# emmanuel-marty/zultra

Hardware: NVIDIA B200
Metric: input MB/s (zultra compression hot path, byte-identical to CPU zultra) (higher is better)
Workload: dtype u8

## Files before the change

### zultra_b200/csrc/zb_pipeline.h

```cpp
#ifndef ZB_PIPELINE_H
#define ZB_PIPELINE_H
#include "zb_rt.h"
#include <vector>
#include <algorithm>
#ifndef ZB_EMU
#include <cuda_pipeline.h>
#endif

#ifndef ZB_CG
#define ZB_CG 1024
#endif
#ifndef ZB_CP
#define ZB_CP 1024
#endif
#define ZB_CD 2048
#define ZB_WU 384
#define ZB_TOKI 256
#define ZB_NH 320
#define ZB_MAXSB 64
#define ZB_MAXNODES 64
#define ZB_MF_TILE_MAX 16384

struct ZbWinDesc {
   uint32_t in_off;
// ... 129 lines not shown
struct ZbPipe {
   zb_stream_t st;
   ZbHostBuf hin, hout;
#ifndef ZB_EMU
   ZbStager stager;
   int device = 0;
#endif
   int nwin = 0, nstream = 0;
   uint32_t P = 0;
   std::vector<ZbWinDesc> h_win;
   std::vector<uint32_t> h_wbase;
   ZbBuf<ZbWinDesc> win; ZbBuf<uint32_t> wbase;
   ZbBuf<uint8_t> in;
   const uint8_t *in_ptr = 0;
   ZbBuf<uint64_t> keyA, keyB; ZbBuf<uint32_t> valA, valB, rank, sa, actA, actB, tmpA, tmpB, scratch;
   ZbBuf<uint32_t> sa_lcp;
   ZbBuf<uint32_t> counters;
   ZbBuf<ZbTileDesc> tiles, units, groups; ZbBuf<uint32_t> tile_iv, tile_pd, tile_cnt, tile_q, unit_words, unit_cnt, group_words, group_cnt, filt_seg;
   ZbBuf<zb_match_t> match; ZbBuf<uint16_t> glen, goff;
   ZbBuf<uint16_t> exitoff, exitc; ZbBuf<uint32_t> gentry, gtokcnt, gtokbase, tokpos, wtok;
   ZbBuf<uint32_t> wtokbase, wintbase; ZbBuf<int> ph;
   std::vector<uint32_t> h_gchunk_first; ZbBuf<uint32_t> gchunk_first, gchunk_win;
   ZbBuf<ZbNode> nodesA, nodesB; ZbBuf<int> nodehist; ZbBuf<uint16_t> chk_stat; ZbBuf<uint8_t> chk_flag; ZbBuf<int> chk_delta; ZbBuf<uint32_t> chk_node;
   ZbBuf<uint32_t> wsplit; ZbBuf<uint32_t> wnsplit, wsubcnt, wsubbase;
   ZbBuf<ZbSub> sub; ZbBuf<ZbSubTabs> tabs; ZbBuf<uint32_t> dchunk_sub, pchunk_sub;
   ZbBuf<zb_match_t> best; ZbBuf<int16_t> sig_true, sig_warm, sig_new; ZbBuf<uint8_t> dok; ZbBuf<uint32_t> dbad;
   ZbBuf<uint32_t> pentry, pbits, cand ; ZbBuf<uint16_t> dpfar;
   int cp = ZB_CP;
   ZbBuf<int> dreach;
   ZbBuf<uint32_t> out; ZbBuf<ZbStreamOut> sout;
   std::vector<ZbStreamOut> h_sout;
   int nsub = 0;
   bool sa_exact = false;
   int parse_cd = 0, parse_wu = ZB_WU;
   int mf_ts_min = ZB_TS_MIN, mf_ts_mul = ZB_TS_MUL;
   int stat_sa_rounds = 0, stat_redo = 0, stat_ub = 0, stat_tiles = 0;
   double t_stage[8];

   void release_all();
   void setup(const std::vector<ZbWinDesc> &wins, const uint8_t *h_in, size_t in_bytes, bool in_is_device);
   void stage_sa();
   void stage_match(uint32_t tile_main);
   void stage_greedy();
   void stage_split();
   void stage_parse();
   void stage_emit(const std::vector<ZbStreamOut> &streams) { stage_emit_prepare(); stage_emit_finish(streams); }
   void stage_emit_prepare();
   void stage_emit_finish(const std::vector<ZbStreamOut> &streams, uint32_t *ext_words = 0);
   void phase_maps(const std::vector<ZbStreamOut> &streams, unsigned long long *bits_out);
   std::vector<ZbStreamOut> plan;
   ZbBuf<uint32_t> ck_tab, ck_part; ZbBuf<uint64_t> ck_rng; bool ck_tab_ready = false;
   void stage_checksum(int kind, const std::vector<uint64_t> &range_off, const std::vector<uint64_t> &range_len, std::vector<uint32_t> &sums, uint32_t init_first);
};

ZB_HD int zb_find_win(const uint32_t *wbase, int nwin, uint32_t g) {
   int lo = 0, hi = nwin - 1;
   while (lo < hi) { int mid = (lo + hi + 1) >> 1; if (wbase[mid] <= g) lo = mid; else hi = mid - 1; }
   return lo;
}

inline void ZbPipe::setup(const std::vector<ZbWinDesc> &wins, const uint8_t *h_in, size_t in_bytes, bool in_is_device) {
   h_win = wins; nwin = (int)wins.size();
   h_wbase.assign(nwin + 1, 0);
   for (int w = 0; w < nwin; w++) h_wbase[w + 1] = h_wbase[w] + wins[w].len;
   P = h_wbase[nwin];
   win.need(nwin); wbase.need(nwin + 1); counters.need(64);
   if (!in_is_device) in.need(in_bytes + 16);
   if (zb_failed()) return;
   zb_h2d(st, win.p, h_win.data(), sizeof(ZbWinDesc) * nwin);
   zb_h2d(st, wbase.p, h_wbase.data(), 4 * (nwin + 1));
   if (in_is_device) in_ptr = h_in;
   else {
      if (h_in) {
#ifndef ZB_EMU
         if (in_bytes >= ((size_t)8 << 20) && ZbStager::pageable(h_in)) { zb_sync(st); if (!stager.copy(0, in.p, (void *)h_in, in_bytes, device)) zb_cuda_fail(cudaErrorUnknown); }
         else
#endif
         zb_h2d(st, in.p, h_in, in_bytes);
      }
      in_ptr = in.p;
   }
}

#define ZB_SA_LOCAL 32

ZB_HD void zb_sa_key(const uint8_t *t, uint32_t i, uint32_t len, uint32_t d, uint64_t &w, uint32_t &tl) {
   const uint32_t rem = len - i;
   tl = rem < d + 9 ? rem : d + 9;
#ifdef __CUDA_ARCH__
   if ((uint64_t)i + d + 12 <= len) {
      const uintptr_t a = (uintptr_t)(t + i + d);
      const uint32_t *pa = (const uint32_t *)(a & ~(uintptr_t)3);
      const uint32_t sh = (uint32_t)(a & 3) << 3;
      const uint32_t x0 = __funnelshift_r(pa[0], pa[1], sh), x1 = __funnelshift_r(pa[1], pa[2], sh);
      w = ((uint64_t)__byte_perm(x0, 0, 0x0123) << 32) | __byte_perm(x1, 0, 0x0123);
      return;
   }
#endif
   uint64_t x = 0;
   for (uint32_t b = 0; b < 8; b++) x = (x << 8) | ((uint64_t)i + d + b < len ? t[i + d + b] : 0u);
   w = x;
}

inline void ZbPipe::stage_sa() {
   const long n = P;
   keyA.need(n); keyB.need(n); valA.need(n); valB.need(n); rank.need(n); sa.need(n); actA.need(n); actB.need(n); tmpA.need(n + 1); tmpB.need(n + 1);
   sa_lcp.need(n);
   scratch.need(zb_sort_scratch_words(n) + zb_scan_scratch_words(n) + 64);
   if (zb_failed()) return;
   int wb = 0; while ((1L << wb) < nwin) wb++;
   int nbytes = (64 - wb) / 8; if (nbytes > 7) nbytes = 7;
   {
      static const int nb_env = getenv("ZULTRA_CUDA_SA_NBYTES") ? atoi(getenv("ZULTRA_CUDA_SA_NBYTES")) : 0;
      if (nb_env >= 3 && nb_env < nbytes) nbytes = nb_env;
   }
   const uint8_t *T = in_ptr; const ZbWinDesc *wd = win.p; const uint32_t *wbs = wbase.p; const int nw = nwin;
   uint64_t *kA = keyA.p; uint32_t *vA = valA.p;
   zb_tag("sa_keys");
   zb_launch(st, n, ZB_LAMBDA(long g) {
      int w = zb_find_win(wbs, nw, (uint32_t)g);
      uint32_t i = (uint32_t)g - wbs[w], len = wd[w].len;
      const uint8_t *t = T + wd[w].in_off;
      uint64_t k = 0;
      for (int b = 0; b < nbytes; b++) k = (k << 8) | (i + b < len ? t[i + b] : 0);
      kA[g] = ((uint64_t)w << (8 * nbytes)) | k;
      vA[g] = (uint32_t)g;
   }, 256);
   zb_sort_pairs(st, keyA.p, valA.p, keyB.p, valB.p, n, 0, 8 * nbytes + wb, scratch.p);
   uint32_t *head = tmpA.p, *grp = tmpB.p, *rk = rank.p, *SA = sa.p, *act = actA.p, *act2 = actB.p, *cnt = counters.p;
   const int kbits = 8 * nbytes;
   zb_tag("sa_group");
   zb_launch(st, n, ZB_LAMBDA(long jl) {
      const uint32_t j = (uint32_t)jl;
      const uint64_t key = kA[j];
      uint32_t gh = j, step = 1;
      while (gh >= step && kA[gh - step] == key) { gh -= step; step <<= 1; }
      long lo = gh >= step ? (long)(gh - step) : -1L;
      while ((long)gh - lo > 1) { const uint32_t mid = (uint32_t)((lo + (long)gh) >> 1); if (kA[mid] == key) gh = mid; else lo = mid; }
      const uint32_t g = vA[j];
      if ((long)gh + ZB_SA_LOCAL < n && kA[gh + ZB_SA_LOCAL] == key) { SA[j] = g; rk[g] = gh; head[j] = 1u; return; }
      uint32_t ge = j + 1;
      while ((long)ge < n && kA[ge] == key) ge++;
      if (ge - gh == 1) { SA[j] = g; rk[g] = j; head[j] = 0u; return; }
      const int w = (int)(key >> kbits);
      const uint32_t base = wbs[w], len = wd[w].len;
      const uint8_t *t = T + wd[w].in_off;
      uint64_t kw; uint32_t kt;
      zb_sa_key(t, g - base, len, (uint32_t)nbytes, kw, kt);
      uint32_t less = 0, eq_before = 0, eq = 0;
      for (uint32_t y = gh; y < ge; y++) {
         if (y == j) continue;
         uint64_t yw; uint32_t yt;
         zb_sa_key(t, vA[y] - base, len, (uint32_t)nbytes, yw, yt);
         if (yw < kw || (yw == kw && yt < kt)) less++;
         else if (yw == kw && yt == kt) { eq++; if (y < j) eq_before++; }
      }
      const uint32_t p = gh + less + eq_before;
      SA[p] = g; rk[g] = gh + less; head[p] = eq ? 1u : 0u;
   }, 256);
   zb_exclusive_sum(st, head, grp, n, cnt, scratch.p);
   zb_launch(st, n, ZB_LAMBDA(long j) { if (head[j]) act[grp[j]] = (uint32_t)j; }, 256);
   uint32_t m = 0;
   zb_d2h(st, &m, cnt, 4); zb_sync(st);
   int rank_bits = 1; while ((1L << rank_bits) < n) rank_bits++;
   uint64_t *kB = keyB.p; uint32_t *vB = valB.p;
   stat_sa_rounds = 0;
   uint32_t maxwin = 0;
   for (int w = 0; w < nwin; w++) maxwin = std::max(maxwin, h_win[w].len);
   int r2_bits = 1; while ((1L << r2_bits) < (long)maxwin + 512) r2_bits++;
   const bool packed_keys = !sa_exact;
   for (uint32_t h = (uint32_t)nbytes; m > 0 && (sa_exact || h < ZB_MAX_MATCH); h <<= 1) {
      stat_sa_rounds++;
      const long mm = m;
      zb_tag("sa_round_keys");
      if (packed_keys) {
         zb_launch(st, mm, ZB_LAMBDA(long a) {
            uint32_t j = act[a], g = SA[j];
            int w = zb_find_win(wbs, nw, g);
            uint32_t wend = wbs[w + 1];
            uint32_t r2;
            if ((uint64_t)g + h < wend) r2 = (rk[g + h] - wbs[w]) + 512u;
            else r2 = wend - g;
            kA[a] = ((uint64_t)rk[g] << r2_bits) | r2;
            vA[a] = g;
         }, 256);
         zb_sort_pairs(st, keyA.p, valA.p, keyB.p, valB.p, mm, 0, r2_bits + rank_bits, scratch.p);
      } else {
      zb_launch(st, mm, ZB_LAMBDA(long a) {
         uint32_t j = act[a], g = SA[j];
         int w = zb_find_win(wbs, nw, g);
         uint32_t wend = wbs[w + 1];
         uint32_t r2;
         if ((uint64_t)g + h < wend) r2 = (rk[g + h] - wbs[w]) + (1u << 22);
         else r2 = wend - g;
         kA[a] = ((uint64_t)rk[g] << 32) | r2;
         vA[a] = g;
      }, 256);
      zb_sort_pairs(st, keyA.p, valA.p, keyB.p, valB.p, mm, 0, 23, scratch.p);
      zb_sort_pairs(st, keyA.p, valA.p, keyB.p, valB.p, mm, 32, 32 + rank_bits, scratch.p);
      }
      zb_launch(st, mm, ZB_LAMBDA(long a) { head[a] = (a == 0 || kA[a] != kA[a - 1]) ? (uint32_t)a : 0u; SA[act[a]] = vA[a]; }, 256);
      zb_inclusive_max(st, head, grp, mm, scratch.p);
      zb_launch(st, mm, ZB_LAMBDA(long a) {
         const uint32_t ga = grp[a];
         rk[vA[a]] = act[ga];
         bool is_head = ga == (uint32_t)a;
         bool next_head = (a + 1 == mm) || grp[a + 1] == (uint32_t)(a + 1);
         head[a] = (is_head && next_head) ? 0u : 1u;
      }, 256);
      zb_exclusive_sum(st, head, (uint32_t *)kB, mm, cnt, scratch.p);
      {
         const uint32_t *dst = (const uint32_t *)kB;
         zb_launch(st, mm, ZB_LAMBDA(long a) { if (head[a]) act2[dst[a]] = act[a]; }, 256);
      }
      zb_d2h(st, &m, cnt, 4); zb_sync(st);
      std::swap(act, act2);
      (void)vB;
      if (h > (1u << 23)) break;
   }
   uint32_t *out = sa_lcp.p;
   zb_tag("lcp_pack");
   zb_launch(st, n, ZB_LAMBDA(long j) {
      uint32_t g = SA[j];
      int w = zb_find_win(wbs, nw, (uint32_t)j);
      uint32_t base = wbs[w], len = wd[w].len;
      uint32_t i = g - base;
      uint32_t l = 0;
      if ((uint32_t)j != base) {
         uint32_t q = SA[j - 1] - base;
         const uint8_t *t = T + wd[w].in_off;
         uint32_t lim = len - (i > q ? i : q);
         if (lim > ZB_MAX_MATCH) lim = ZB_MAX_MATCH;
#ifdef __CUDA_ARCH__
         if (wd[w].in_off + (i < q ? i : q) >= 4) {
            while (l + 8 <= lim) {
               const uintptr_t a = (uintptr_t)(t + i + l), b = (uintptr_t)(t + q + l);
               const uint32_t *pa = (const uint32_t *)(a & ~(uintptr_t)3), *pb = (const uint32_t *)(b & ~(uintptr_t)3);
               const uint32_t x = __funnelshift_r(pa[0], pa[1], (uint32_t)(a & 3) << 3) ^ __funnelshift_r(pb[0], pb[1], (uint32_t)(b & 3) << 3);
               if (x) { l += (uint32_t)(__ffs((int)x) - 1) >> 3; lim = l; break; }
               l += 4;
            }
         }
// ... 2655 lines not shown
```

### zultra_b200/csrc/zb_prims.cu

```cuda
#include "zb_rt.h"

void zb_cuda_fail(cudaError_t e) {
   (void)e;
   g_zb_cuda_error = 1;
}
thread_local int g_zb_cuda_error = 0;
long long g_zb_launches = 0;

#include <vector>
#include <string>
#include <map>
#include <mutex>
int g_zb_prof_on = 0;
struct ZbProfRec { std::string tag; cudaEvent_t a, b; };
static std::vector<ZbProfRec> g_prof;
static std::mutex g_prof_mu;
static thread_local const char *g_next_tag = 0;
static thread_local ZbProfRec g_cur;
void zb_tag(const char *tag) { g_next_tag = tag; }
void zb_prof_begin(int line, cudaStream_t st) {
   if (g_next_tag) g_cur.tag = g_next_tag; else { char b[32]; snprintf(b, sizeof b, "L%d", line); g_cur.tag = b; }
   g_next_tag = 0;
   cudaEventCreate(&g_cur.a); cudaEventCreate(&g_cur.b);
   cudaEventRecord(g_cur.a, st);
// ... 195 lines not shown
      __syncwarp();
   }
   __syncthreads();
   uint32_t tot = 0;
#pragma unroll
   for (int w = 0; w < RS_WARPS; w++) { uint32_t t = cnt[w][tid]; cnt[w][tid] = tot; tot += t; }
   uint32_t inc = tot;
#pragma unroll
   for (int d = 1; d < 32; d <<= 1) { uint32_t o = __shfl_up_sync(0xffffffffu, inc, d); if (lane >= d) inc += o; }
   if (lane == 31) wsum[warp] = inc;
   __syncthreads();
   uint32_t woff = 0;
#pragma unroll
   for (int w = 0; w < RS_WARPS; w++) if (w < warp) woff += wsum[w];
   const uint32_t ds = woff + inc - tot;
   dstart[tid] = ds;
   gbase[tid] = gb - ds;
   __syncthreads();
#pragma unroll
   for (int k = 0; k < RS_ITEMS; k++) {
      const long idx = base + k * 32 + lane;
      if (idx < n) {
         const uint32_t d = (uint32_t)(key[k] >> shift) & mask;
         const uint32_t lp = dstart[d] + cnt[warp][d] + rk[k];
         skey[lp] = key[k]; sval[lp] = val[k];
      }
   }
   __syncthreads();
   const long tile_n = n - (long)blockIdx.x * RS_TILE < RS_TILE ? n - (long)blockIdx.x * RS_TILE : RS_TILE;
#pragma unroll
   for (int k = 0; k < RS_ITEMS; k++) {
      const int e = k * RS_THREADS + tid;
      if (e < tile_n) {
         const uint64_t kk = skey[e];
         const uint32_t d = (uint32_t)(kk >> shift) & mask;
         const size_t dst = (size_t)(uint32_t)(gbase[d] + (uint32_t)e);
         kout[dst] = kk;
         vout[dst] = sval[e];
      }
   }
}

size_t zb_sort_scratch_words(long n) {
   long ntiles = (n + RS_TILE - 1) / RS_TILE;
   if (ntiles < 1) ntiles = 1;
   return (size_t)256 * ntiles + zb_scan_scratch_words(256 * ntiles) + 64;
}

void zb_sort_pairs(zb_stream_t st, uint64_t *keys, uint32_t *vals, uint64_t *keys_tmp, uint32_t *vals_tmp, long n, int bit_lo, int bit_hi, uint32_t *scratch) {
   if (n <= 1 || bit_hi <= bit_lo) return;
   const int ntiles = (int)((n + RS_TILE - 1) / RS_TILE);
   uint32_t *hist = scratch;
   uint32_t *scan_scratch = scratch + (size_t)256 * ntiles;
   uint64_t *kin = keys, *kout = keys_tmp;
   uint32_t *vin = vals, *vout = vals_tmp;
   int npass = 0;
   for (int shift = bit_lo; shift < bit_hi; shift += 8, npass++) {
      const int w = (bit_hi - shift) < 8 ? (bit_hi - shift) : 8;
      const uint32_t mask = (1u << w) - 1u;
      PROF_K("rs_hist", st);
      rs_hist_k<<<ntiles, RS_THREADS, 0, st>>>(kin, n, shift, mask, hist, ntiles);
      PROF_E(st);
      scan_impl<OpSum, false>(st, hist, hist, (long)256 * ntiles, 0, scan_scratch);
      PROF_K("rs_scatter", st);
      rs_scatter_k<<<ntiles, RS_THREADS, 0, st>>>(kin, vin, kout, vout, n, shift, mask, hist, ntiles);
      PROF_E(st);
      zb_count_launch(2);
      uint64_t *tk = kin; kin = kout; kout = tk;
      uint32_t *tv = vin; vin = vout; vout = tv;
   }
   ZB_CUDA_CHECK(cudaGetLastError());
   if (npass & 1) {
      ZB_CUDA_CHECK(cudaMemcpyAsync(keys, keys_tmp, (size_t)n * 8, cudaMemcpyDeviceToDevice, st));
      ZB_CUDA_CHECK(cudaMemcpyAsync(vals, vals_tmp, (size_t)n * 4, cudaMemcpyDeviceToDevice, st));
   }
}


#define DS_SEG 4096
#define DS_THREADS 256
#define DS_WORDS (DS_SEG / 32)
#define DS_BROW (DS_WORDS + 1)
#define DS_PROW (DS_WORDS + 2)

__device__ __forceinline__ int ds_find_win(const ZbDistWin *dw, int nwin, uint32_t seg) {
   int lo = 0, hi = nwin - 1;
   while (lo < hi) { const int mid = (lo + hi + 1) >> 1; if (dw[mid].seg_base <= seg) lo = mid; else hi = mid - 1; }
   return lo;
}

template <bool SCATTER>
__global__ void __launch_bounds__(DS_THREADS) unit_dist_k(const uint32_t *sa_lcp, const ZbDistWin *dw, int nwin, int nu_max, uint32_t *segrec, uint32_t *unit_words) {
   extern __shared__ uint32_t ds_sm[];
   uint32_t *bm = ds_sm;
   uint16_t *pre = (uint16_t *)(bm + (size_t)nu_max * DS_BROW);
   uint16_t *lcp = pre + (size_t)nu_max * DS_PROW;
   uint16_t *bmin = lcp + DS_SEG;
   uint32_t *uoff = (uint32_t *)(bmin + DS_WORDS);
   uint32_t *stage = uoff + nu_max + 1;
   const int tid = threadIdx.x, lane = tid & 31, warp = tid >> 5;
   const int w = ds_find_win(dw, nwin, blockIdx.x);
   const ZbDistWin W = dw[w];
   const uint32_t seg = blockIdx.x - W.seg_base, r0 = seg * DS_SEG;
   const uint32_t nr = W.len - r0 < DS_SEG ? W.len - r0 : DS_SEG;
   const int nu = (int)W.nu;
   {
      const size_t tot = (size_t)dw[nwin - 1].sa_base + dw[nwin - 1].len;
      const size_t pf = (size_t)W.sa_base + r0 + (size_t)1024 * DS_SEG + (size_t)tid * 32;
      if (tid < DS_SEG / 32 && pf < tot) asm volatile("prefetch.global.L2 [%0];" :: "l"(sa_lcp + pf));
   }
   if (nu == 1) {
      if (!SCATTER) { if (tid == 0) { segrec[(size_t)blockIdx.x * nu_max * 2] = nr; segrec[(size_t)blockIdx.x * nu_max * 2 + 1] = 0x1ffu | 0x10000u; } }
      else for (uint32_t idx = tid; idx < nr; idx += DS_THREADS) unit_words[(size_t)W.unit_base * (2 * ZB_MAX_OFFSET) + r0 + idx] = __ldg(sa_lcp + W.sa_base + r0 + idx);
      return;
   }
   uint32_t wv[DS_SEG / DS_THREADS];
#pragma unroll
   for (int k = 0; k < DS_SEG / DS_THREADS; k++) {
      const uint32_t idx = (uint32_t)k * DS_THREADS + tid;
      wv[k] = idx < nr ? __ldg(sa_lcp + W.sa_base + r0 + idx) : (0x1ffu << ZB_POS_BITS);
   }
   for (int e = tid; e < nu * DS_BROW; e += DS_THREADS) bm[e] = 0;
   __syncthreads();
#pragma unroll
   for (int k = 0; k < DS_SEG / DS_THREADS; k++) {
      const uint32_t idx = (uint32_t)k * DS_THREADS + tid;
      uint32_t v = wv[k];
      if (idx < nr) {
         const uint32_t p = v & ZB_POS_MASK;
         const int ua = p < W.hist ? 0 : (int)((p - W.hist) >> 15);
         atomicOr(bm + ua * DS_BROW + (idx >> 5), 1u << (idx & 31));
         if (p >= W.hist && ua + 1 < nu) atomicOr(bm + (ua + 1) * DS_BROW + (idx >> 5), 1u << (idx & 31));
      }
      wv[k] = v;
      lcp[idx] = (uint16_t)((v >> ZB_POS_BITS) & 0x1ffu);
   }
   __syncthreads();
   for (int b = warp; b < DS_WORDS; b += DS_THREADS / 32) {
      const uint32_t m = __reduce_min_sync(0xffffffffu, (uint32_t)lcp[b * 32 + lane]);
      if (lane == 0) bmin[b] = (uint16_t)m;
   }
   __syncthreads();
   uint32_t *rec = segrec + (size_t)blockIdx.x * nu_max * 2;
   if (!SCATTER) {
      for (int u = warp; u < nu; u += DS_THREADS / 32) {
         const uint32_t *b = bm + u * DS_BROW;
         uint32_t c = 0; int last = -1;
#pragma unroll
         for (int j = 0; j < DS_WORDS / 32; j++) {
            const uint32_t x = b[j * 32 + lane];
            c += (uint32_t)__popc(x);
            if (x) last = (j * 32 + lane) * 32 + 31 - __clz((int)x);
         }
#pragma unroll
         for (int d = 16; d > 0; d >>= 1) { c += __shfl_xor_sync(0xffffffffu, c, d); last = max(last, __shfl_xor_sync(0xffffffffu, last, d)); }
         uint32_t m = 0x1ffu;
         const int from = last + 1;
         const int fb = (from + 31) >> 5;
         { const int i = from + lane; if (i < fb * 32 && i < DS_SEG) m = lcp[i]; }
         for (int bb = fb + lane; bb < DS_WORDS; bb += 32) m = min(m, (uint32_t)bmin[bb]);
         m = __reduce_min_sync(0xffffffffu, m);
         if (lane == 0) { rec[2 * u] = c; rec[2 * u + 1] = m | (last >= 0 ? 0x10000u : 0u); }
      }
      return;
   }
   for (int u = warp; u < nu; u += DS_THREADS / 32) {
      const uint32_t *b = bm + u * DS_BROW;
      uint32_t run = 0;
#pragma unroll
      for (int j = 0; j < DS_WORDS / 32; j++) {
         const uint32_t c = (uint32_t)__popc(b[j * 32 + lane]);
         uint32_t inc = c;
#pragma unroll
         for (int d = 1; d < 32; d <<= 1) { const uint32_t o = __shfl_up_sync(0xffffffffu, inc, d); if (lane >= d) inc += o; }
         pre[u * DS_PROW + j * 32 + lane] = (uint16_t)(run + inc - c);
         run += __shfl_sync(0xffffffffu, inc, 31);
      }
      if (lane == 0) uoff[u + 1] = run;
   }
   __syncthreads();
   if (tid == 0) { uint32_t acc = 0; uoff[0] = 0; for (int u = 0; u < nu; u++) { const uint32_t c = uoff[u + 1]; uoff[u + 1] = acc + c; acc += c; } }
   __syncthreads();
#pragma unroll
   for (int k = 0; k < DS_SEG / DS_THREADS; k++) {
      const uint32_t idx = (uint32_t)k * DS_THREADS + tid;
      if (idx >= nr) continue;
      const uint32_t p = wv[k] & ZB_POS_MASK;
      const int ua = p < W.hist ? 0 : (int)((p - W.hist) >> 15);
      const int nun = (p >= W.hist && ua + 1 < nu) ? 2 : 1;
      for (int q = 0; q < nun; q++) {
         const int u = ua + q;
         const uint32_t *b = bm + u * DS_BROW;
         const uint32_t wi = idx >> 5, below = b[wi] & ((1u << (idx & 31)) - 1u);
         const uint32_t rank = (uint32_t)pre[u * DS_PROW + wi] + (uint32_t)__popc(below);
         int prev = -1;
         if (below) prev = (int)(wi * 32) + 31 - __clz((int)below);
         else for (int x = (int)wi - 1; x >= 0; x--) { const uint32_t y = b[x]; if (y) { prev = x * 32 + 31 - __clz((int)y); break; } }
         uint32_t m = 0x1ffu;
         const int from = prev + 1, fb = (from + 31) >> 5, lb = (int)(idx >> 5);
         if (fb > lb) { for (int i = from; i <= (int)idx; i++) m = min(m, (uint32_t)lcp[i]); }
         else {
            for (int i = from; i < fb * 32; i++) m = min(m, (uint32_t)lcp[i]);
            for (int bb = fb; bb < lb; bb++) m = min(m, (uint32_t)bmin[bb]);
            for (int i = lb * 32; i <= (int)idx; i++) m = min(m, (uint32_t)lcp[i]);
         }
         if (prev < 0) m = min(m, rec[2 * u + 1]);
         const uint32_t m0 = W.hist + (uint32_t)u * ZB_MAX_OFFSET, ulo = m0 > ZB_MAX_OFFSET ? m0 - ZB_MAX_OFFSET : 0;
         stage[uoff[u] + rank] = (p - ulo) | (m << ZB_POS_BITS);
      }
   }
   __syncthreads();
   for (int u = warp; u < nu; u += DS_THREADS / 32) {
      const uint32_t a = uoff[u], n = uoff[u + 1] - a;
      uint32_t *dst = unit_words + (size_t)(W.unit_base + u) * (2 * ZB_MAX_OFFSET) + rec[2 * u];
      for (uint32_t j = lane; j < n; j += 32) dst[j] = stage[a + j];
   }
}

__global__ void unit_dist_offsets_k(const ZbDistWin *dw, int nwin, int nu_max, uint32_t *segrec, uint32_t *unit_cnt, int total_units) {
   const int g = blockIdx.x * blockDim.x + threadIdx.x;
   if (g >= total_units) return;
   int lo = 0, hi = nwin - 1;
   while (lo < hi) { const int mid = (lo + hi + 1) >> 1; if (dw[mid].unit_base <= (uint32_t)g) lo = mid; else hi = mid - 1; }
   const ZbDistWin W = dw[lo];
   const int u = g - (int)W.unit_base;
   const uint32_t nseg = (W.len + DS_SEG - 1) / DS_SEG;
   uint32_t acc = 0, carry = 0x1ffu;
   for (uint32_t sg = 0; sg < nseg; sg++) {
      uint32_t *rec = segrec + ((size_t)(W.seg_base + sg) * nu_max + u) * 2;
      const uint32_t c = rec[0], th = rec[1];
      rec[0] = acc; rec[1] = carry;
      acc += c;
      const uint32_t tl = th & 0xffffu;
      carry = (th >> 16) ? tl : (tl < carry ? tl : carry);
   }
   unit_cnt[g] = acc;
}

void zb_unit_distribute(zb_stream_t st, const uint32_t *sa_lcp, const ZbDistWin *dw, int nwin, int nseg_total, int total_units, int nu_max, uint32_t *segrec,
                        uint32_t *unit_words, uint32_t *unit_cnt) {
   if (nseg_total <= 0 || total_units <= 0) return;
   const size_t smem = (size_t)nu_max * DS_BROW * 4 + (size_t)nu_max * DS_PROW * 2 + DS_SEG * 2 + DS_WORDS * 2 + ((size_t)nu_max + 1) * 4 + 2 * DS_SEG * 4 + 16;
   ZB_CUDA_CHECK(cudaFuncSetAttribute(unit_dist_k<false>, cudaFuncAttributeMaxDynamicSharedMemorySize, 112 * 1024));
   ZB_CUDA_CHECK(cudaFuncSetAttribute(unit_dist_k<true>, cudaFuncAttributeMaxDynamicSharedMemorySize, 112 * 1024));
   PROF_K("mf_unit_dist", st);
   unit_dist_k<false><<<nseg_total, DS_THREADS, smem - 2 * DS_SEG * 4, st>>>(sa_lcp, dw, nwin, nu_max, segrec, unit_words);
   unit_dist_offsets_k<<<(total_units + 127) / 128, 128, 0, st>>>(dw, nwin, nu_max, segrec, unit_cnt, total_units);
   unit_dist_k<true><<<nseg_total, DS_THREADS, smem, st>>>(sa_lcp, dw, nwin, nu_max, segrec, unit_words);
   PROF_E(st);
   zb_count_launch(3);
   ZB_CUDA_CHECK(cudaGetLastError());
}
```

Measured before the change: 1507.

## Resolve small suffix-array groups in shared memory with multi-step local refinement

```diff
diff --git a/zultra_b200/csrc/zb_pipeline.h b/zultra_b200/csrc/zb_pipeline.h
--- a/zultra_b200/csrc/zb_pipeline.h
+++ b/zultra_b200/csrc/zb_pipeline.h
@@ -235,7 +235,9 @@
    }
 }
 
-#define ZB_SA_LOCAL 32
+#define ZB_SA_LOCAL 64
+#define ZB_SA_SPAN 1024
+#define ZB_SA_STEPS 2
 
 ZB_HD void zb_sa_key(const uint8_t *t, uint32_t i, uint32_t len, uint32_t d, uint64_t &w, uint32_t &tl) {
    const uint32_t rem = len - i;
@@ -254,6 +256,197 @@
    for (uint32_t b = 0; b < 8; b++) x = (x << 8) | ((uint64_t)i + d + b < len ? t[i + d + b] : 0u);
    w = x;
 }
+
+#ifndef ZB_EMU
+struct ZbSaRec { uint64_t w; uint32_t st; uint32_t g; };
+#define ZB_SA_LT 256
+#define ZB_SA_CAP (ZB_SA_SPAN + ZB_SA_LOCAL - 1)
+#define ZB_SA_SPT (ZB_SA_SPAN / ZB_SA_LT)
+#define ZB_SA_IPT ((ZB_SA_CAP + ZB_SA_LT - 1) / ZB_SA_LT)
+
+__device__ __forceinline__ bool zb_sa_rec_less(const ZbSaRec &a, const ZbSaRec &b) {
+   if ((a.st >> 9) != (b.st >> 9)) return a.st < b.st;
+   if (a.w != b.w) return a.w < b.w;
+   return a.st < b.st;
+}
+
+template <bool MAX> __device__ __forceinline__ uint32_t zb_sa_cta_scan(uint32_t v, uint32_t *ws, uint32_t &tot) {
+   const int lane = threadIdx.x & 31, warp = threadIdx.x >> 5;
+   uint32_t inc = v;
+#pragma unroll
+   for (int o = 1; o < 32; o <<= 1) { const uint32_t y = __shfl_up_sync(0xffffffffu, inc, o); if (lane >= o) inc = MAX ? max(inc, y) : inc + y; }
+   uint32_t ex = __shfl_up_sync(0xffffffffu, inc, 1);
+   if (lane == 0) ex = 0;
+   if (lane == 31) ws[warp] = inc;
+   __syncthreads();
+   uint32_t pre = 0, all = 0;
+#pragma unroll
+   for (int w = 0; w < ZB_SA_LT / 32; w++) {
+      const uint32_t x = ws[w];
+      if (w < warp) pre = MAX ? max(pre, x) : pre + x;
+      all = MAX ? max(all, x) : all + x;
+   }
+   __syncthreads();
+   tot = all;
+   return MAX ? max(pre, ex) : pre + ex;
+}
+
+__global__ void __launch_bounds__(ZB_SA_LT) zb_sa_local_k(const uint64_t *kA, const uint32_t *vA, long n, const uint8_t *T, const ZbWinDesc *wd,
+                                                         const uint32_t *wbs, int nw, uint32_t nb, uint32_t *SA, uint32_t *rk, uint32_t *head) {
+   extern __shared__ __align__(16) ZbSaRec zb_sar[];
+   ZbSaRec *A = zb_sar, *B = zb_sar + ZB_SA_CAP;
+   uint16_t *pos = (uint16_t *)(zb_sar + 2 * ZB_SA_CAP);
+   uint16_t *grp = pos + ZB_SA_CAP;
+   __shared__ uint32_t ws[ZB_SA_LT / 32], s_end, s_tail;
+   const int tid = threadIdx.x;
+   const uint32_t s0 = blockIdx.x * ZB_SA_SPAN, s1 = (uint32_t)min((long)s0 + ZB_SA_SPAN, n);
+   __shared__ uint16_t gsz[ZB_SA_SPAN];
+   __shared__ uint8_t gstart[ZB_SA_SPAN];
+   __shared__ uint32_t s_gh0, s_large0;
+   const uint32_t sl = s1 - s0, p0 = tid * ZB_SA_SPT;
+   for (int p = tid; p < ZB_SA_CAP; p += ZB_SA_LT) grp[p] = 0xffffu;
+   if (tid == 0) {
+      s_end = sl; s_tail = 0xffffu; s_gh0 = s0; s_large0 = 0;
+      const uint64_t key = kA[s0];
+      if (s0 > 0 && kA[s0 - 1] == key) {
+         uint32_t gh = s0, step = 1;
+         while (gh >= step && kA[gh - step] == key) { gh -= step; step <<= 1; }
+         long lo = gh >= step ? (long)(gh - step) : -1L;
+         while ((long)gh - lo > 1) { const uint32_t mid = (uint32_t)((lo + (long)gh) >> 1); if (kA[mid] == key) gh = mid; else lo = mid; }
+         s_gh0 = gh; s_large0 = (long)gh + ZB_SA_LOCAL < n && kA[gh + ZB_SA_LOCAL] == key;
+      }
+   }
+   uint64_t key[ZB_SA_SPT];
+   uint32_t startm = 0, last_start = 0;
+#pragma unroll
+   for (int i = 0; i < ZB_SA_SPT; i++) {
+      const uint32_t p = p0 + i, j = s0 + p;
+      key[i] = p < sl ? kA[j] : 0;
+      const bool st = p < sl && (j == 0 || (i ? key[i - 1] : kA[j - 1]) != key[i]);
+      gstart[p] = st;
+      if (st) { startm |= 1u << i; last_start = p + 1; }
+   }
+   uint32_t unused;
+   uint32_t cur = zb_sa_cta_scan<true>(last_start, ws, unused);
+#pragma unroll
+   for (int i = 0; i < ZB_SA_SPT; i++) {
+      if (!((startm >> i) & 1u)) continue;
+      const uint32_t p = p0 + i, lim = min(p + ZB_SA_LOCAL + 1, sl);
+      uint32_t q = p + 1;
+      while (q < lim && !gstart[q]) q++;
+      uint32_t sz = q - p;
+      if (q == p + ZB_SA_LOCAL + 1) sz = ZB_SA_LOCAL + 1;
+      else if (q == sl && (long)s1 < n && kA[s1] == key[i]) {
+         const uint32_t gh = s0 + p;
+         if ((long)gh + ZB_SA_LOCAL < n && kA[gh + ZB_SA_LOCAL] == key[i]) sz = ZB_SA_LOCAL + 1;
+         else {
+            uint32_t e = s1, st2 = 1;
+            while ((long)e + st2 < n && kA[e + st2] == key[i]) { e += st2; st2 <<= 1; }
+            long hi = min((long)e + st2, n);
+            while (hi - (long)e > 1) { const uint32_t mid = (uint32_t)(((long)e + hi) >> 1); if (kA[mid] == key[i]) e = mid; else hi = mid; }
+            sz = (uint32_t)hi - gh; s_end = (uint32_t)hi - s0; s_tail = p;
+         }
+      }
+      gsz[p] = (uint16_t)sz;
+   }
+   __syncthreads();
+#pragma unroll
+   for (int i = 0; i < ZB_SA_SPT; i++) {
+      const uint32_t p = p0 + i, j = s0 + p;
+      if (p >= sl) break;
+      if ((startm >> i) & 1u) cur = p + 1;
+      const uint32_t g = vA[j];
+      if (cur == 0) {
+         if (s_large0) { SA[j] = g; rk[g] = s_gh0; head[j] = 1u; }
+         continue;
+      }
+      const uint32_t sz = gsz[cur - 1], gh = s0 + cur - 1;
+      if (sz > ZB_SA_LOCAL) { SA[j] = g; rk[g] = gh; head[j] = 1u; }
+      else if (sz == 1) { SA[j] = g; rk[g] = j; head[j] = 0u; }
+      else grp[p] = (uint16_t)(cur - 1);
+   }
+   __syncthreads();
+   const uint32_t np = s_end;
+   for (uint32_t p = sl + tid; p < np; p += ZB_SA_LT) grp[p] = (uint16_t)s_tail;
+   __syncthreads();
+   uint32_t na;
+   {
+      uint32_t c = 0;
+#pragma unroll
+      for (int i = 0; i < ZB_SA_IPT; i++) { const uint32_t p = tid * ZB_SA_IPT + i; if (p < np && grp[p] != 0xffffu) c++; }
+      uint32_t o = zb_sa_cta_scan<false>(c, ws, na);
+#pragma unroll
+      for (int i = 0; i < ZB_SA_IPT; i++) {
+         const uint32_t p = tid * ZB_SA_IPT + i;
+         if (p < np && grp[p] != 0xffffu) { A[o].w = 0; A[o].st = (uint32_t)grp[p] << 9; A[o].g = vA[s0 + p]; pos[o] = (uint16_t)p; o++; }
+      }
+      __syncthreads();
+   }
+   for (uint32_t d = nb, step = 0; na > 0; d += 8, step++) {
+      for (uint32_t k = tid; k < na; k += ZB_SA_LT) {
+         ZbSaRec &r = A[k];
+         const int w = zb_find_win(wbs, nw, r.g);
+         uint64_t kw; uint32_t tl;
+         zb_sa_key(T + wd[w].in_off, r.g - wbs[w], wd[w].len, d, kw, tl);
+         r.w = kw; r.st = (r.st & ~511u) | tl;
+      }
+      __syncthreads();
+      for (uint32_t k = tid; k < na; k += ZB_SA_LT) {
+         const ZbSaRec r = A[k];
+         const uint32_t run = r.st >> 9;
+         uint32_t lo = k;
+         while (lo > 0 && (A[lo - 1].st >> 9) == run) lo--;
+         uint32_t before = 0;
+         for (uint32_t y = lo; y < na && (A[y].st >> 9) == run; y++) {
+            const ZbSaRec x = A[y];
+            before += zb_sa_rec_less(x, r) || (y < k && x.w == r.w && x.st == r.st);
+         }
+         B[lo + before] = r;
+      }
+      __syncthreads();
+      { ZbSaRec *t = A; A = B; B = t; }
+      const bool last = step + 1 == ZB_SA_STEPS;
+      const uint32_t full = d + 9;
+      uint32_t run_last = 0, ntied = 0, tpm = 0, tnm = 0;
+#pragma unroll
+      for (int i = 0; i < ZB_SA_IPT; i++) {
+         const uint32_t k = tid * ZB_SA_IPT + i;
+         if (k < na) {
+            const ZbSaRec r = A[k];
+            const bool tied = (r.st & 511u) == full;
+            const bool tp = tied && k > 0 && A[k - 1].st == r.st && A[k - 1].w == r.w;
+            const bool tn = tied && k + 1 < na && A[k + 1].st == r.st && A[k + 1].w == r.w;
+            if (!tp) run_last = k;
+            if (tp || tn) ntied++;
+            tpm |= (uint32_t)tp << i; tnm |= (uint32_t)tn << i;
+         }
+      }
+      uint32_t unused, nt;
+      uint32_t rs = zb_sa_cta_scan<true>(run_last, ws, unused);
+      uint32_t o = zb_sa_cta_scan<false>(last ? 0u : ntied, ws, nt);
+      uint32_t kg[ZB_SA_IPT]; uint16_t kp[ZB_SA_IPT], kr[ZB_SA_IPT];
+#pragma unroll
+      for (int i = 0; i < ZB_SA_IPT; i++) {
+         const uint32_t k = tid * ZB_SA_IPT + i;
+         kg[i] = 0xffffffffu;
+         if (k < na) {
+            if (!((tpm >> i) & 1u)) rs = k;
+            const uint32_t g = A[k].g, slot = s0 + pos[k], rslot = s0 + pos[rs];
+            const bool tied = ((tpm | tnm) >> i) & 1u;
+            if (!tied) { SA[slot] = g; rk[g] = slot; head[slot] = 0u; }
+            else if (last) { SA[slot] = g; rk[g] = rslot; head[slot] = 1u; }
+            else { kg[i] = g; kp[i] = pos[k]; kr[i] = pos[rs]; }
+         }
+      }
+      __syncthreads();
+#pragma unroll
+      for (int i = 0; i < ZB_SA_IPT; i++)
+         if (kg[i] != 0xffffffffu) { A[o].w = 0; A[o].st = (uint32_t)kr[i] << 9; A[o].g = kg[i]; pos[o] = kp[i]; o++; }
+      __syncthreads();
+      na = last ? 0u : nt;
+   }
+}
+#endif
 
 inline void ZbPipe::stage_sa() {
    const long n = P;
@@ -281,36 +474,54 @@
    }, 256);
    zb_sort_pairs(st, keyA.p, valA.p, keyB.p, valB.p, n, 0, 8 * nbytes + wb, scratch.p);
    uint32_t *head = tmpA.p, *grp = tmpB.p, *rk = rank.p, *SA = sa.p, *act = actA.p, *act2 = actB.p, *cnt = counters.p;
-   const int kbits = 8 * nbytes;
-   zb_tag("sa_group");
-   zb_launch(st, n, ZB_LAMBDA(long jl) {
-      const uint32_t j = (uint32_t)jl;
-      const uint64_t key = kA[j];
-      uint32_t gh = j, step = 1;
-      while (gh >= step && kA[gh - step] == key) { gh -= step; step <<= 1; }
-      long lo = gh >= step ? (long)(gh - step) : -1L;
-      while ((long)gh - lo > 1) { const uint32_t mid = (uint32_t)((lo + (long)gh) >> 1); if (kA[mid] == key) gh = mid; else lo = mid; }
-      const uint32_t g = vA[j];
-      if ((long)gh + ZB_SA_LOCAL < n && kA[gh + ZB_SA_LOCAL] == key) { SA[j] = g; rk[g] = gh; head[j] = 1u; return; }
-      uint32_t ge = j + 1;
-      while ((long)ge < n && kA[ge] == key) ge++;
-      if (ge - gh == 1) { SA[j] = g; rk[g] = j; head[j] = 0u; return; }
-      const int w = (int)(key >> kbits);
-      const uint32_t base = wbs[w], len = wd[w].len;
-      const uint8_t *t = T + wd[w].in_off;
-      uint64_t kw; uint32_t kt;
-      zb_sa_key(t, g - base, len, (uint32_t)nbytes, kw, kt);
-      uint32_t less = 0, eq_before = 0, eq = 0;
-      for (uint32_t y = gh; y < ge; y++) {
-         if (y == j) continue;
-         uint64_t yw; uint32_t yt;
-         zb_sa_key(t, vA[y] - base, len, (uint32_t)nbytes, yw, yt);
-         if (yw < kw || (yw == kw && yt < kt)) less++;
-         else if (yw == kw && yt == kt) { eq++; if (y < j) eq_before++; }
-      }
-      const uint32_t p = gh + less + eq_before;
-      SA[p] = g; rk[g] = gh + less; head[p] = eq ? 1u : 0u;
-   }, 256);
+#ifndef ZB_EMU
+   {
+      const size_t smem = (size_t)ZB_SA_CAP * (2 * sizeof(ZbSaRec) + 4);
+      ZB_CUDA_CHECK(cudaFuncSetAttribute(zb_sa_local_k, cudaFuncAttributeMaxDynamicSharedMemorySize, (int)smem));
+      if (g_zb_prof_on) { zb_tag("sa_local"); zb_prof_begin(0, st); }
+      zb_sa_local_k<<<(unsigned)((n + ZB_SA_SPAN - 1) / ZB_SA_SPAN), ZB_SA_LT, smem, st>>>(kA, vA, n, T, wd, wbs, nw, (uint32_t)nbytes, SA, rk, head);
+      if (g_zb_prof_on) zb_prof_end(st);
+      zb_count_launch(1);
+      ZB_CUDA_CHECK(cudaGetLastError());
+   }
+#else
+   {
+      struct Rec { uint64_t w; uint32_t tl, g; bool operator<(const Rec &o) const { return w != o.w ? w < o.w : tl != o.tl ? tl < o.tl : g < o.g; } };
+      const int kbits = 8 * nbytes;
+      std::vector<Rec> r;
+      std::vector<std::pair<uint32_t, uint32_t>> runs, next;
+      for (uint32_t gh = 0, ge; (long)gh < n; gh = ge) {
+         for (ge = gh + 1; (long)ge < n && kA[ge] == kA[gh]; ge++) {}
+         const bool large = ge - gh > ZB_SA_LOCAL;
+         for (uint32_t j = gh; j < ge; j++) { SA[j] = vA[j]; rk[vA[j]] = ge - gh == 1 ? j : gh; head[j] = large ? 1u : 0u; }
+         if (large || ge - gh == 1) continue;
+         const int w = (int)(kA[gh] >> kbits);
+         runs.assign(1, std::make_pair(gh, ge));
+         for (uint32_t d = (uint32_t)nbytes, step = 0; !runs.empty(); d += 8, step++) {
+            const bool last = step + 1 == ZB_SA_STEPS;
+            next.clear();
+            for (const auto &ab : runs) {
+               r.clear();
+               for (uint32_t j = ab.first; j < ab.second; j++) {
+                  Rec x; x.g = SA[j];
+                  zb_sa_key(T + wd[w].in_off, x.g - wbs[w], wd[w].len, d, x.w, x.tl);
+                  r.push_back(x);
+               }
+               std::sort(r.begin(), r.end());
+               for (uint32_t i = 0, e; i < r.size(); i = e) {
+                  for (e = i + 1; e < r.size() && r[e].w == r[i].w && r[e].tl == r[i].tl && r[i].tl == d + 9; e++) {}
+                  for (uint32_t q = i; q < e; q++) {
+                     const uint32_t slot = ab.first + q;
+                     SA[slot] = r[q].g; rk[r[q].g] = ab.first + i; head[slot] = e - i > 1 && last ? 1u : 0u;
+                  }
+                  if (e - i > 1 && !last) next.push_back(std::make_pair(ab.first + i, ab.first + e));
+               }
+            }
+            runs.swap(next);
+         }
+      }
+   }
+#endif
    zb_exclusive_sum(st, head, grp, n, cnt, scratch.p);
    zb_launch(st, n, ZB_LAMBDA(long j) { if (head[j]) act[grp[j]] = (uint32_t)j; }, 256);
    uint32_t m = 0;
```

After: 1495, median of 6. About the same (-0.8%).

## Replace serial LCP range-min scans with warp-level sparse-table and segmented scans

Applied to the files above, without the earlier changes.

```diff
diff --git a/zultra_b200/csrc/zb_prims.cu b/zultra_b200/csrc/zb_prims.cu
--- a/zultra_b200/csrc/zb_prims.cu
+++ b/zultra_b200/csrc/zb_prims.cu
@@ -301,6 +301,7 @@
 #define DS_WORDS (DS_SEG / 32)
 #define DS_BROW (DS_WORDS + 1)
 #define DS_PROW (DS_WORDS + 2)
+#define DS_SROW 33
 
 __device__ __forceinline__ int ds_find_win(const ZbDistWin *dw, int nwin, uint32_t seg) {
    int lo = 0, hi = nwin - 1;
@@ -308,15 +309,28 @@
    return lo;
 }
 
+__device__ __forceinline__ uint32_t ds_lane_range_min(const uint32_t (&win)[6], int a, int lane) {
+   const int k = 31 - __clz(lane - a + 1);
+   uint32_t m = 0;
+#pragma unroll
+   for (int j = 0; j < 6; j++) {
+      const uint32_t o = __shfl_sync(0xffffffffu, win[j], (a + (1 << j) - 1) & 31);
+      if (j == k) m = min(win[j], o);
+   }
+   return m;
+}
+
 template <bool SCATTER>
 __global__ void __launch_bounds__(DS_THREADS) unit_dist_k(const uint32_t *sa_lcp, const ZbDistWin *dw, int nwin, int nu_max, uint32_t *segrec, uint32_t *unit_words) {
    extern __shared__ uint32_t ds_sm[];
-   uint32_t *bm = ds_sm;
+   uint16_t *smin = (uint16_t *)ds_sm;
+   uint16_t *bmin = smin + DS_WORDS * DS_SROW;
+   uint32_t *ucnt = (uint32_t *)(bmin + DS_WORDS);
+   int *ulast = (int *)(ucnt + nu_max + 1);
+   uint32_t *bm = (uint32_t *)(ulast + nu_max);
    uint16_t *pre = (uint16_t *)(bm + (size_t)nu_max * DS_BROW);
-   uint16_t *lcp = pre + (size_t)nu_max * DS_PROW;
-   uint16_t *bmin = lcp + DS_SEG;
-   uint32_t *uoff = (uint32_t *)(bmin + DS_WORDS);
-   uint32_t *stage = uoff + nu_max + 1;
+   uint16_t *gap = pre + (size_t)nu_max * DS_PROW;
+   uint32_t *stage = (uint32_t *)(gap + (size_t)nu_max * DS_PROW);
    const int tid = threadIdx.x, lane = tid & 31, warp = tid >> 5;
    const int w = ds_find_win(dw, nwin, blockIdx.x);
    const ZbDistWin W = dw[w];
@@ -339,98 +353,108 @@
       const uint32_t idx = (uint32_t)k * DS_THREADS + tid;
       wv[k] = idx < nr ? __ldg(sa_lcp + W.sa_base + r0 + idx) : (0x1ffu << ZB_POS_BITS);
    }
-   for (int e = tid; e < nu * DS_BROW; e += DS_THREADS) bm[e] = 0;
+   if (SCATTER) { for (int e = tid; e < nu * DS_BROW; e += DS_THREADS) bm[e] = 0; }
+   else { for (int u = tid; u < nu; u += DS_THREADS) { ucnt[u] = 0; ulast[u] = -1; } }
    __syncthreads();
 #pragma unroll
    for (int k = 0; k < DS_SEG / DS_THREADS; k++) {
       const uint32_t idx = (uint32_t)k * DS_THREADS + tid;
-      uint32_t v = wv[k];
-      if (idx < nr) {
-         const uint32_t p = v & ZB_POS_MASK;
-         const int ua = p < W.hist ? 0 : (int)((p - W.hist) >> 15);
-         atomicOr(bm + ua * DS_BROW + (idx >> 5), 1u << (idx & 31));
-         if (p >= W.hist && ua + 1 < nu) atomicOr(bm + (ua + 1) * DS_BROW + (idx >> 5), 1u << (idx & 31));
-      }
-      wv[k] = v;
-      lcp[idx] = (uint16_t)((v >> ZB_POS_BITS) & 0x1ffu);
-   }
-   __syncthreads();
-   for (int b = warp; b < DS_WORDS; b += DS_THREADS / 32) {
-      const uint32_t m = __reduce_min_sync(0xffffffffu, (uint32_t)lcp[b * 32 + lane]);
-      if (lane == 0) bmin[b] = (uint16_t)m;
+      const uint32_t v = wv[k], p = v & ZB_POS_MASK;
+      const int ua = p < W.hist ? 0 : (int)((p - W.hist) >> 15);
+      const bool in = idx < nr, dual = p >= W.hist && ua + 1 < nu;
+      if (SCATTER) {
+         if (in) {
+            atomicOr(bm + ua * DS_BROW + (idx >> 5), 1u << lane);
+            if (dual) atomicOr(bm + (ua + 1) * DS_BROW + (idx >> 5), 1u << lane);
+         }
+      } else {
+#pragma unroll
+         for (int q = 0; q < 2; q++) {
+            const int u = in && (q == 0 || dual) ? ua + q : -1;
+            const uint32_t peers = __match_any_sync(0xffffffffu, (uint32_t)u);
+            if (u >= 0 && lane == 31 - __clz((int)peers)) { atomicAdd(ucnt + u, (uint32_t)__popc(peers)); atomicMax(ulast + u, (int)idx); }
+         }
+      }
+      uint32_t s = (v >> ZB_POS_BITS) & 0x1ffu;
+#pragma unroll
+      for (int d = 1; d < 32; d <<= 1) { const uint32_t o = __shfl_down_sync(0xffffffffu, s, d); if (lane + d < 32) s = min(s, o); }
+      smin[(idx >> 5) * DS_SROW + lane] = (uint16_t)s;
+      if (lane == 0) bmin[idx >> 5] = (uint16_t)s;
    }
    __syncthreads();
    uint32_t *rec = segrec + (size_t)blockIdx.x * nu_max * 2;
    if (!SCATTER) {
       for (int u = warp; u < nu; u += DS_THREADS / 32) {
-         const uint32_t *b = bm + u * DS_BROW;
-         uint32_t c = 0; int last = -1;
-#pragma unroll
-         for (int j = 0; j < DS_WORDS / 32; j++) {
-            const uint32_t x = b[j * 32 + lane];
-            c += (uint32_t)__popc(x);
-            if (x) last = (j * 32 + lane) * 32 + 31 - __clz((int)x);
-         }
-#pragma unroll
-         for (int d = 16; d > 0; d >>= 1) { c += __shfl_xor_sync(0xffffffffu, c, d); last = max(last, __shfl_xor_sync(0xffffffffu, last, d)); }
-         uint32_t m = 0x1ffu;
-         const int from = last + 1;
-         const int fb = (from + 31) >> 5;
-         { const int i = from + lane; if (i < fb * 32 && i < DS_SEG) m = lcp[i]; }
+         const int last = ulast[u], from = last + 1, fb = (from + 31) >> 5;
+         uint32_t m = lane == 0 && (from & 31) ? (uint32_t)smin[(from >> 5) * DS_SROW + (from & 31)] : 0x1ffu;
          for (int bb = fb + lane; bb < DS_WORDS; bb += 32) m = min(m, (uint32_t)bmin[bb]);
          m = __reduce_min_sync(0xffffffffu, m);
-         if (lane == 0) { rec[2 * u] = c; rec[2 * u + 1] = m | (last >= 0 ? 0x10000u : 0u); }
+         if (lane == 0) { rec[2 * u] = ucnt[u]; rec[2 * u + 1] = m | (last >= 0 ? 0x10000u : 0u); }
       }
       return;
    }
    for (int u = warp; u < nu; u += DS_THREADS / 32) {
       const uint32_t *b = bm + u * DS_BROW;
-      uint32_t run = 0;
+      uint32_t run = 0, gin = rec[2 * u + 1];
 #pragma unroll
       for (int j = 0; j < DS_WORDS / 32; j++) {
-         const uint32_t c = (uint32_t)__popc(b[j * 32 + lane]);
+         const int wd = j * 32 + lane;
+         const uint32_t x = b[wd];
+         const uint32_t c = (uint32_t)__popc(x);
          uint32_t inc = c;
 #pragma unroll
          for (int d = 1; d < 32; d <<= 1) { const uint32_t o = __shfl_up_sync(0xffffffffu, inc, d); if (lane >= d) inc += o; }
-         pre[u * DS_PROW + j * 32 + lane] = (uint16_t)(run + inc - c);
+         pre[u * DS_PROW + wd] = (uint16_t)(run + inc - c);
          run += __shfl_sync(0xffffffffu, inc, 31);
-      }
-      if (lane == 0) uoff[u + 1] = run;
-   }
-   __syncthreads();
-   if (tid == 0) { uint32_t acc = 0; uoff[0] = 0; for (int u = 0; u < nu; u++) { const uint32_t c = uoff[u + 1]; uoff[u + 1] = acc + c; acc += c; } }
+         const int t = 32 - __clz((int)x);
+         uint32_t f = x != 0, g = x == 0 ? (uint32_t)bmin[wd] : t < 32 ? (uint32_t)smin[wd * DS_SROW + t] : 0x1ffu;
+#pragma unroll
+         for (int d = 1; d < 32; d <<= 1) {
+            const uint32_t fo = __shfl_up_sync(0xffffffffu, f, d), go = __shfl_up_sync(0xffffffffu, g, d);
+            if (lane >= d) { if (!f) g = min(g, go); f |= fo; }
+         }
+         const uint32_t incl = f ? g : min(gin, g);
+         const uint32_t excl = __shfl_up_sync(0xffffffffu, incl, 1);
+         gap[u * DS_PROW + wd] = (uint16_t)(lane == 0 ? gin : excl);
+         gin = __shfl_sync(0xffffffffu, incl, 31);
+      }
+      if (lane == 0) ucnt[u + 1] = run;
+   }
+   __syncthreads();
+   if (tid == 0) { uint32_t acc = 0; ucnt[0] = 0; for (int u = 0; u < nu; u++) { const uint32_t c = ucnt[u + 1]; ucnt[u + 1] = acc + c; acc += c; } }
    __syncthreads();
 #pragma unroll
    for (int k = 0; k < DS_SEG / DS_THREADS; k++) {
-      const uint32_t idx = (uint32_t)k * DS_THREADS + tid;
-      if (idx >= nr) continue;
-      const uint32_t p = wv[k] & ZB_POS_MASK;
+      const uint32_t idx = (uint32_t)k * DS_THREADS + tid, wi = idx >> 5;
+      const uint32_t v = wv[k], p = v & ZB_POS_MASK;
       const int ua = p < W.hist ? 0 : (int)((p - W.hist) >> 15);
-      const int nun = (p >= W.hist && ua + 1 < nu) ? 2 : 1;
-      for (int q = 0; q < nun; q++) {
+      const bool in = idx < nr, dual = p >= W.hist && ua + 1 < nu;
+      uint32_t win[6];
+      win[0] = (v >> ZB_POS_BITS) & 0x1ffu;
+#pragma unroll
+      for (int j = 1; j < 6; j++) { const uint32_t o = __shfl_up_sync(0xffffffffu, win[j - 1], 1 << (j - 1)); win[j] = lane >= (1 << (j - 1)) ? min(win[j - 1], o) : win[j - 1]; }
+#pragma unroll
+      for (int q = 0; q < 2; q++) {
+         const bool on = in && (q == 0 || dual);
          const int u = ua + q;
-         const uint32_t *b = bm + u * DS_BROW;
-         const uint32_t wi = idx >> 5, below = b[wi] & ((1u << (idx & 31)) - 1u);
-         const uint32_t rank = (uint32_t)pre[u * DS_PROW + wi] + (uint32_t)__popc(below);
-         int prev = -1;
-         if (below) prev = (int)(wi * 32) + 31 - __clz((int)below);
-         else for (int x = (int)wi - 1; x >= 0; x--) { const uint32_t y = b[x]; if (y) { prev = x * 32 + 31 - __clz((int)y); break; } }
-         uint32_t m = 0x1ffu;
-         const int from = prev + 1, fb = (from + 31) >> 5, lb = (int)(idx >> 5);
-         if (fb > lb) { for (int i = from; i <= (int)idx; i++) m = min(m, (uint32_t)lcp[i]); }
-         else {
-            for (int i = from; i < fb * 32; i++) m = min(m, (uint32_t)lcp[i]);
-            for (int bb = fb; bb < lb; bb++) m = min(m, (uint32_t)bmin[bb]);
-            for (int i = lb * 32; i <= (int)idx; i++) m = min(m, (uint32_t)lcp[i]);
+         uint32_t rank = 0, g = 0x1ffu;
+         int a = lane;
+         if (on) {
+            const uint32_t below = bm[u * DS_BROW + wi] & ((1u << lane) - 1u);
+            rank = (uint32_t)pre[u * DS_PROW + wi] + (uint32_t)__popc(below);
+            if (below) a = 32 - __clz((int)below);
+            else { a = 0; g = gap[u * DS_PROW + wi]; }
          }
-         if (prev < 0) m = min(m, rec[2 * u + 1]);
-         const uint32_t m0 = W.hist + (uint32_t)u * ZB_MAX_OFFSET, ulo = m0 > ZB_MAX_OFFSET ? m0 - ZB_MAX_OFFSET : 0;
-         stage[uoff[u] + rank] = (p - ulo) | (m << ZB_POS_BITS);
+         const uint32_t m = min(g, ds_lane_range_min(win, a, lane));
+         if (on) {
+            const uint32_t m0 = W.hist + (uint32_t)u * ZB_MAX_OFFSET, ulo = m0 > ZB_MAX_OFFSET ? m0 - ZB_MAX_OFFSET : 0;
+            stage[ucnt[u] + rank] = (p - ulo) | (m << ZB_POS_BITS);
+         }
       }
    }
    __syncthreads();
    for (int u = warp; u < nu; u += DS_THREADS / 32) {
-      const uint32_t a = uoff[u], n = uoff[u + 1] - a;
+      const uint32_t a = ucnt[u], n = ucnt[u + 1] - a;
       uint32_t *dst = unit_words + (size_t)(W.unit_base + u) * (2 * ZB_MAX_OFFSET) + rec[2 * u];
       for (uint32_t j = lane; j < n; j += 32) dst[j] = stage[a + j];
    }
@@ -459,11 +483,12 @@
 void zb_unit_distribute(zb_stream_t st, const uint32_t *sa_lcp, const ZbDistWin *dw, int nwin, int nseg_total, int total_units, int nu_max, uint32_t *segrec,
                         uint32_t *unit_words, uint32_t *unit_cnt) {
    if (nseg_total <= 0 || total_units <= 0) return;
-   const size_t smem = (size_t)nu_max * DS_BROW * 4 + (size_t)nu_max * DS_PROW * 2 + DS_SEG * 2 + DS_WORDS * 2 + ((size_t)nu_max + 1) * 4 + 2 * DS_SEG * 4 + 16;
-   ZB_CUDA_CHECK(cudaFuncSetAttribute(unit_dist_k<false>, cudaFuncAttributeMaxDynamicSharedMemorySize, 112 * 1024));
-   ZB_CUDA_CHECK(cudaFuncSetAttribute(unit_dist_k<true>, cudaFuncAttributeMaxDynamicSharedMemorySize, 112 * 1024));
+   const size_t smem_count = (size_t)DS_WORDS * DS_SROW * 2 + DS_WORDS * 2 + ((size_t)nu_max + 1) * 4 + (size_t)nu_max * 4;
+   const size_t smem = smem_count + (size_t)nu_max * DS_BROW * 4 + (size_t)nu_max * DS_PROW * 2 * 2 + 2 * DS_SEG * 4;
+   ZB_CUDA_CHECK(cudaFuncSetAttribute(unit_dist_k<false>, cudaFuncAttributeMaxDynamicSharedMemorySize, (int)smem_count));
+   ZB_CUDA_CHECK(cudaFuncSetAttribute(unit_dist_k<true>, cudaFuncAttributeMaxDynamicSharedMemorySize, (int)smem));
    PROF_K("mf_unit_dist", st);
-   unit_dist_k<false><<<nseg_total, DS_THREADS, smem - 2 * DS_SEG * 4, st>>>(sa_lcp, dw, nwin, nu_max, segrec, unit_words);
+   unit_dist_k<false><<<nseg_total, DS_THREADS, smem_count, st>>>(sa_lcp, dw, nwin, nu_max, segrec, unit_words);
    unit_dist_offsets_k<<<(total_units + 127) / 128, 128, 0, st>>>(dw, nwin, nu_max, segrec, unit_cnt, total_units);
    unit_dist_k<true><<<nseg_total, DS_THREADS, smem, st>>>(sa_lcp, dw, nwin, nu_max, segrec, unit_words);
    PROF_E(st);
```

Measured after the change: 1506 before, 1552 after, median of 6. 1.03x the previous value.
